# truongchauhien/CUDA.RadixSort

Measured on AMD Instinct MI355X. Metric: Mkeys/s sorting 2^30 uniform uint32; scatter-pass achieved HBM GB/s, higher is better.
Workload: dtype u32; 1 GPU; sort 1073741824 uint32 keys per GPU, k=8 (4 passes), uniform; keys_per_gpu=1073741824, k_bits=8, passes=4, dist=uniform, pairs=False, rank_algo=match, tile_keys=16384, tiles_per_chunk=256, num_chunks=256, parallelism=single GPU

## Files before the change

cuda.radixsort_amd/csrc/rsort_capi.cpp:

```cpp
#include <hip/hip_runtime.h>
#include <stdint.h>
#include <stdlib.h>
#include <string.h>

#include <math.h>

#include <algorithm>
#include <atomic>
#include <mutex>
#include <vector>

#include "rsort.h"
#include "rsort_internal.hpp"

using namespace rsort;

namespace {

constexpr int kVersion = 100;
std::atomic<int> g_rank_algo{RSORT_RANK_MATCH};
std::atomic<int> g_group_chunks{1};
std::atomic<int> g_table_fault{0};
std::atomic<int> g_rank_fault{0};
std::atomic<int> g_hybrid{RSORT_HYBRID_AUTO};
// ... 352 lines not shown
    a.kout = kout;
    a.vout = vout;
    a.table = table;
    a.n = (uint64_t)p.n;
    a.chunk_keys = (uint64_t)p.chunk_keys;
    a.num_chunks = (uint32_t)p.num_chunks;
    a.shift = (uint32_t)shift;
    a.local_only = local_only ? 1u : 0u;
    a.nsplit = (uint32_t)nsplit;
    for (int i = 0; i < nsplit; ++i) a.splitters[i] = split[i];
    const int rank = internal_rank((dmode == kDigitShift) ? g_rank_algo.load() : RSORT_RANK_MATCH);
    const int geom = geom_from_shape(p.threads, p.tile_keys, p.pairs);
    if (!scatter_available(p.k_bits, p.pairs, rank, dmode, geom)) return RSORT_ERR_ARG;
    const int aligned16 = line_capable(kout, vout, p.pairs, p.n);
    if ((bounds || next_table || raw_table) && !(rank == kRankAtomic && aligned16 && !local_only && dmode == kDigitShift))
        return RSORT_ERR_ARG;
    PhaseScope ps(dmode == kDigitSplit ? RSORT_PHASE_PARTITION : RSORT_PHASE_SCATTER, p.n, s, gate);
    return hip_status(launch_scatter(p.k_bits, p.pairs, rank, dmode, geom, local_only ? 0 : aligned16, a, s));
}

int check_plan(const rsort_plan *p) {
    if (!p) return RSORT_ERR_ARG;
    if (p->k_bits < kMinBits || p->k_bits > kMaxBits) return RSORT_ERR_BITS;
    if (p->n < 0 || p->n >= ((int64_t)1 << 32)) return RSORT_ERR_SIZE;
    if (geom_from_shape(p->threads, p->tile_keys, p->pairs) < 0) return RSORT_ERR_ARG;
    if (p->tiles_per_chunk <= 0 || p->num_chunks <= 0 ||
        p->num_chunks * p->tiles_per_chunk * p->tile_keys < p->n ||
        p->chunk_keys != p->tiles_per_chunk * p->tile_keys || p->bins != (1 << p->k_bits) ||
        p->table_entries != (int64_t)p->bins * p->num_chunks)
        return RSORT_ERR_ARG;
    return RSORT_OK;
}

constexpr int64_t kHybMinKeys = (int64_t)3 << 28;
constexpr int64_t kHybMaxKeys = (int64_t)kHybCapacity * kHybBuckets;
int64_t hyb_min_keys() {
    static const int64_t v = [] {
        const char *e = lab_env("RSORT_HYB_MIN_KEYS");
        const long long x = e ? atoll(e) : 0;
        return (x >= 1 && x < ((long long)1 << 32)) ? (int64_t)x : kHybMinKeys;
    }();
    return v;
}

constexpr int kHybGridMult = 4;

uint32_t gate_threshold(int64_t n) {
    const double m = (double)std::min<int64_t>(n, kHybSample) / (double)kHybGateGroups;
    const double lam = m * std::max(1.0 / (double)kHybBuckets, (double)kHybCapacity / (double)std::max<int64_t>(n, 1));
    double lp = -lam;
    for (uint32_t k = 0; k < 65535u; ++k) {
        if ((double)(k + 1) > lam) {
            const double tail = exp(lp) / (1.0 - lam / (double)(k + 1));
            if (tail * (double)kHybBuckets * (double)kHybGateGroups < 1e-9) return std::max(k, 2u);
        }
        lp += log(lam) - log((double)(k + 1));
    }
    return 65535u;
}

bool hybrid_eligible(const rsort_plan &p, bool joint, bool inplace, bool allow) {
    const int hm = g_hybrid.load();
    if (!allow || hm == RSORT_HYBRID_OFF || !joint || p.pairs || inplace || p.passes != 4) return false;
    if (hm == RSORT_HYBRID_FORCE) return true;
    return p.n >= hyb_min_keys() && p.n <= kHybMaxKeys;
}

int sort_planned(const rsort_plan &p, const uint32_t *kin, const uint32_t *vin, uint32_t *kout,
                 uint32_t *vout, void *ws, size_t wsb, hipStream_t s, bool allow_hybrid = true) {
    int st = check_plan(&p);
    if (st) return st;
    if (p.n == 0) return RSORT_OK;
    if (!kin || !kout || !ws || (p.pairs && (!vin || !vout))) return RSORT_ERR_ARG;
    if (!aligned4(kin) || !aligned4(kout) || (p.pairs && (!aligned4(vin) || !aligned4(vout))))
        return RSORT_ERR_ALIGN;
    if (wsb < p.workspace_bytes) return RSORT_ERR_WORKSPACE;
    const Carve c = carve(p, ws);
    const int P = p.passes;
// ... 32 lines not shown
        h.kin = kin;
        h.kout = kout;
        h.joint = c.joint;
        h.bounds = hb;
        h.gflags = c.bounds;
        h.done = c.done;
        h.n = (uint64_t)p.n;
        h.threshold = gate_threshold(p.n);
        h.force = force ? 1u : 0u;
        h.rank_fault = g_rank_fault.load() ? 1u : 0u;
        hyb_note_bucket();
        {
            PhaseScope ps(RSORT_PHASE_HISTOGRAM, std::min<int64_t>(p.n, kHybSample), s);
            if (hipMemsetAsync(c.joint, 0, (size_t)kJointBins * kJointBins * 4 + 16, s) != hipSuccess) return RSORT_ERR_HIP;
            if ((st = hip_status(launch_hyb_gate(h, s)))) return st;
        }
        if ((st = do_histogram_joint(p, kin, 24, c.table, c.joint, nullptr, s, false, nullptr, nullptr, nullptr, 16,
                                     g_try)))
            return st;
        {
            PhaseScope ps(RSORT_PHASE_HISTOGRAM, p.n, s);
            if ((st = hip_status(launch_hyb_bounds(h, s)))) return st;
        }
        if ((st = do_scan(p, c.table, c.bsums, s, nullptr, nullptr, nullptr, nullptr, g_run))) return st;
        if ((st = do_scatter(p, kin, nullptr, kout, nullptr, 24, c.table, 0, kDigitShift, nullptr, 0, s, nullptr,
                             nullptr, nullptr, nullptr, nullptr, 0, nullptr, c.done + kDoneErr, g_run)))
            return st;
        if ((st = do_scatter(p, kout, nullptr, c.tmp_k, nullptr, 16, c.joint, 0, kDigitShift, nullptr, 0, s, hb,
                             nullptr, nullptr, nullptr, nullptr, 0, nullptr, c.done + kDoneErr, g_run)))
            return st;
        {
            const int cus = std::max(1, device_cus());
            const int bpc = std::max(1, hyb_blocks_per_cu());
            const uint32_t grid = (uint32_t)std::min<int64_t>(kHybBuckets, (int64_t)cus * bpc * kHybGridMult);
            h.kin = c.tmp_k;
            PhaseScope ps(RSORT_PHASE_SCATTER, p.n, s, g_run);
            if ((st = hip_status(launch_hyb_bucket(h, grid, s)))) return st;
        }
    }
    for (int i = 0; i < P; ++i) {
        const int shift = i * p.k_bits;
        const bool to_out = ((P - 1 - i) % 2) == 0;
        uint32_t *dk = to_out ? kout : c.tmp_k;
        uint32_t *dv = to_out ? vout : c.tmp_v;
        const bool count_joint = joint && (i % 2 == 0) && i + 1 < P;
        const uint32_t *bounds = (joint && (i % 2 == 1)) ? c.bounds + (i / 2) * kBoundsWords : nullptr;
        uint32_t *tab = rawt ? rot[i % 3] : (nextc && (i % 2 == 1)) ? c.table2 : c.table;
        uint32_t *nxt = (nextc && i + 1 < P) ? (rawt ? rot[(i + 1) % 3] : (i % 2 == 1) ? c.table : c.table2) : nullptr;
        uint32_t *clr = (rawt && i + 2 < P) ? rot[(i + 2) % 3] : nullptr;
        const uint32_t *enable = (count_joint && i >= 2) ? c.bounds + (i / 2 - 1) * kBoundsWords : nullptr;
        if (count_joint) {
            if ((st = do_histogram_joint(p, sk, shift, c.table, c.joint, enable, s, i == 0 && !hyb, rows, rows_cnt,
                                         (i == 0 && !hyb) ? c.done : nullptr, 0, lsd)))
                return st;
        } else if (!(nextc && i > 0) &&
                   (st = do_histogram(p, sk, shift, tab, kDigitShift, nullptr, 0, s, bounds, c.joint, c.plan,
                                      c.pcounts, rawt ? nxt : nullptr, i == 0 ? c.done : nullptr,
                                      bounds ? rows : nullptr, lsd))) {
            return st;
        }
        if (!(nextc && i > 0) && !rawt &&
            (st = do_scan(p, tab, c.bsums, s, nxt, nextc ? c.done : nullptr, bounds ? &c : nullptr, bounds, lsd)))
            return st;
        if (count_joint && (st = do_joint_bounds(p, c.joint, enable, c.bounds + (i / 2) * kBoundsWords, c.plan,
                                                 c.pcounts, tab, rows_cnt, rows ? rows + kRowsWords : nullptr, s, lsd)))
            return st;
        const uint32_t *cl = (joint && i >= 1) ? c.bounds + ((i - 1) / 2) * kBoundsWords : nullptr;
// ... 405 lines not shown
    if (!d_keys_in || !d_keys_out || (plan->pairs && (!d_vals_in || !d_vals_out)))
        return RSORT_ERR_ARG;
    if (d_keys_in == d_keys_out) return RSORT_ERR_ARG;
    const uint32_t *table = nullptr;
    return do_scatter(*plan, d_keys_in, d_vals_in, d_keys_out, d_vals_out, shift, table, 1,
                      kDigitShift, nullptr, 0, (hipStream_t)stream);
}

int rsort_set_rank_algo(int algo) {
    if (algo != RSORT_RANK_MATCH && algo != RSORT_RANK_SPLIT && algo != RSORT_RANK_BALLOT) return RSORT_ERR_ARG;
    g_rank_algo.store(algo);
    return RSORT_OK;
}

int rsort_get_rank_algo(void) { return g_rank_algo.load(); }

int rsort_set_group_chunks(int enable) {
    g_group_chunks.store(enable ? 1 : 0);
    return RSORT_OK;
}

int rsort_get_group_chunks(void) { return g_group_chunks.load(); }

int rsort_set_hybrid(int mode) {
    if (mode != RSORT_HYBRID_AUTO && mode != RSORT_HYBRID_OFF && mode != RSORT_HYBRID_FORCE) return RSORT_ERR_ARG;
    g_hybrid.store(mode);
    return RSORT_OK;
}

int rsort_get_hybrid(void) { return g_hybrid.load(); }

int rsort_hybrid_capacity(void) { return (int)kHybCapacity; }

int rsort_hybrid_range(int64_t *min_keys, int64_t *max_keys) {
    if (!min_keys || !max_keys) return RSORT_ERR_ARG;
    *min_keys = hyb_min_keys();
    *max_keys = kHybMaxKeys;
    return RSORT_OK;
}

int rsort_hybrid_gate_threshold(int64_t n) {
    if (n <= 0 || n >= ((int64_t)1 << 32)) return -RSORT_ERR_SIZE;
    return (int)gate_threshold(n);
}

int rsort_hybrid_report(const rsort_plan *plan, const void *d_workspace, int *report, void *stream) {
    if (!plan || !report || !d_workspace) return RSORT_ERR_ARG;
    int st = check_plan(plan);
    if (st) return st;
    for (int i = 0; i < 4; ++i) report[i] = 0;
    if (plan->n == 0) return RSORT_OK;
    const Carve c = carve(*plan, const_cast<void *>(d_workspace));
    hipStream_t s = (hipStream_t)stream;
    uint32_t h[4] = {0, 0, 0, 0};
    if (hipMemcpyAsync(h, c.done + kHybMode, sizeof(h), hipMemcpyDeviceToHost, s) != hipSuccess) return RSORT_ERR_HIP;
    if (hipStreamSynchronize(s) != hipSuccess) return RSORT_ERR_HIP;
    report[0] = (int)h[kHybEligible - kHybMode];
    report[1] = (int)h[kHybGate - kHybMode];
    report[2] = (int)h[kHybMax - kHybMode];
    report[3] = h[0] == kHybRun ? 1 : 0;
    return RSORT_OK;
}

int rsort_group_flags(const rsort_plan *plan, const void *d_workspace, int *flags, void *stream) {
    if (!plan || !flags || !d_workspace) return RSORT_ERR_ARG;
    int st = check_plan(plan);
// ... 269 lines not shown
```

cuda.radixsort_amd/csrc/rsort_hooks.hpp:

```cpp
#pragma once
#include <hip/hip_runtime.h>
#include <stdint.h>

#ifdef RSORT_LAB_HOOKS
#include RSORT_LAB_HOOKS
#else
namespace rsort {
namespace hooks {
constexpr int kDeferKeysCl = 2;
constexpr int kDeferKeysPlain = 0;
constexpr int kDeferPairs = 4;
constexpr int kNextReplicas = 8;
constexpr int kLinesMinWavesSmall = 1;

typedef uint32_t u32x4h __attribute__((ext_vector_type(4)));
__device__ __forceinline__ void store_quad_nt(uint32_t *p, const u32x4h &v) {
    __builtin_nontemporal_store(v, reinterpret_cast<u32x4h *>(p));
}
__device__ __forceinline__ void store_quad(uint32_t *p, const u32x4h &v) { *reinterpret_cast<u32x4h *>(p) = v; }
__device__ __forceinline__ void store_word(uint32_t *p, uint32_t v) { *p = v; }
}
}
#define RS_WG_T0
#define RS_WG_T1
#define RS_WG_TH1
#define RS_STAMP_DECL
#define RS_STAMP(i)
#define RS_STAMP_FLUSH()
#endif
```

cuda.radixsort_amd/csrc/rsort_hybrid.hip:

```cpp
#include <hip/hip_runtime.h>
#include <stdint.h>

#include "rsort_device.hpp"
#include "rsort_hooks.hpp"
#include "rsort_internal.hpp"

namespace rsort {

namespace {

constexpr uint32_t kPadKey = 0xFFFFFFFFu;
typedef uint32_t u32x4 __attribute__((ext_vector_type(4)));

__global__ __launch_bounds__(1024) void rs_hyb_gate(HybArgs a) {
    constexpr uint32_t T = 1024;
    __shared__ uint32_t s_c[kHybBuckets / 2];
    const uint32_t t = threadIdx.x;
    const uint64_t m = a.n < (uint64_t)kHybSample ? a.n : (uint64_t)kHybSample;
    const uint64_t stride = m ? a.n / m : 1;
    const uint64_t i = (uint64_t)blockIdx.x * T + t;
    const uint32_t k = i < m ? __builtin_nontemporal_load(a.kin + i * stride) : 0u;
    for (uint32_t x = t; x < kHybBuckets / 2; x += T) s_c[x] = 0u;
    __syncthreads();
    if (i < m) {
        const uint32_t bk = k >> 16, sh = (bk & 1u) << 4;
        const uint32_t before = (atomicAdd(&s_c[bk >> 1], 1u << sh) >> sh) & 0xFFFFu;
        if (before + 1u >= a.threshold) a.joint[kHybGateFlag] = 1u;
    }
}

__global__ __launch_bounds__(1024) void rs_hyb_bounds(HybArgs a) {
    constexpr uint32_t R = kJointBins, Q = 1024 / R, EP = R / Q;
    __shared__ uint32_t s_part[Q][R];
    __shared__ uint32_t s_start[R];
    __shared__ uint32_t s_ws[1024 / kWave];
    __shared__ uint32_t s_max;
    const uint32_t t = threadIdx.x;
    const bool skew = a.joint[kHybGateFlag] != 0u;
    if (t == 0) {
        a.done[0] = 0u;
        a.done[kDoneErr] = 0u;
        a.done[kHybGate] = skew ? kGateSkewed : kGatePass;
        a.done[kHybEligible] = 1u;
    }
// ... 42 lines not shown
        }
        return;
    }
    if (t < R) {
        s_start[t] = start;
        a.bounds[1 + t] = start;
    }
    if (t == 0) {
        a.bounds[0] = kGroupsWhole;
        a.bounds[1 + R] = total;
    }
    __syncthreads();
    uint32_t run = s_start[g];
    for (uint32_t i = 0; i < q; ++i) run += s_part[i][g];
#pragma unroll 1
    for (uint32_t i0 = 0; i0 < EP; i0 += B) {
        uint32_t v[B];
#pragma unroll
        for (uint32_t i = 0; i < B; ++i) v[i] = col[(i0 + i) * R];
#pragma unroll
        for (uint32_t i = 0; i < B; ++i) {
            col[(i0 + i) * R] = run;
            run += v[i];
        }
    }
    if (t == 0) {
        a.done[kHybMode] = kHybRun;
        a.done[kHybMax] = big;
        a.gflags[0] = kGroupsWhole;
        a.gflags[kBoundsWords] = kGroupsFixed;
    }
}

template <int THREADS, int KPT>
__global__ __launch_bounds__(THREADS) void rs_bucket_sort16(HybArgs a) {
    constexpr int W = THREADS / kWave;
    constexpr uint32_t CAP = THREADS * KPT;
    static_assert(CAP == kHybCapacity && CAP % kWave == 0, "the capacity the exact count checks");
    __shared__ __attribute__((aligned(16))) uint32_t s_k[CAP + 4];
    __shared__ uint32_t s_cnt[W * 256];
    __shared__ uint32_t s_ws[W];
    if (a.done[kHybMode] != kHybRun) return;
    const uint32_t t = threadIdx.x, w = t / kWave, lane = lane_id();
    uint32_t *row = &s_cnt[w * 256];
    uint32_t order_bad = 0, size_bad = 0;
    auto bucket = [&](uint32_t b, uint32_t &s, uint32_t &n) {
        s = 0u;
        n = 0u;
        if (b >= kHybBuckets) return;
        s = a.joint[(b & 255u) * kJointBins + (b >> 8)];
        const uint32_t b1 = b + 1u;
        const uint32_t e = b1 < kHybBuckets ? a.joint[(b1 & 255u) * kJointBins + (b1 >> 8)] : (uint32_t)a.n;
        n = e - s;
        if (e < s || n > CAP || (uint64_t)e > a.n) {
            size_bad = 1u;
            n = 0u;
        }
    };
    auto span_of = [&](uint32_t n) { return ((((n + 63u) / 64u) + W - 1) / W) * 64u; };
    uint32_t key[KPT];
    auto load = [&](uint32_t s, uint32_t n) {
        const uint32_t span = span_of(n), i0 = w * span + lane;
#pragma unroll
        for (int j = 0; j < KPT; ++j) {
            const uint32_t i = i0 + j * kWave;
            const bool in = (uint32_t)(j * kWave) < span && i < n;
            key[j] = in ? __builtin_nontemporal_load(a.kin + s + i) : kPadKey;
        }
    };
    for (uint32_t b = blockIdx.x; b < kHybBuckets; b += gridDim.x) {
        uint32_t s, n;
        bucket(b, s, n);
        load(s, n);
        const uint32_t span = span_of(n), i0 = w * span + lane;
        const uint32_t ak = (uint32_t)(((uintptr_t)(a.kout + s) >> 2) & 3u);
        for (int pass = 0; pass < 2; ++pass) {
            const uint32_t sh = pass * 8;
            for (uint32_t i = lane; i < 256; i += kWave) row[i] = 0;
            uint32_t rk[KPT];
#pragma unroll
            for (int j = 0; j < KPT; ++j) {
                rk[j] = 0;
                if ((uint32_t)(j * kWave) < span && w * span + j * kWave < n) {
                    const uint32_t d = (key[j] >> sh) & 255u;
                    rk[j] = rank_add(row, d);
                    if (j == 0 && w * span + kWave <= n) order_bad |= rank_check<8>(d, rk[j], a.rank_fault);
                }
            }
            __syncthreads();
            uint32_t tot = 0;
            if (t < 256) {
#pragma unroll
                for (int x = 0; x < W; ++x) {
                    const uint32_t c = s_cnt[x * 256 + t];
                    s_cnt[x * 256 + t] = tot;
                    tot += c;
                }
            }
            uint32_t all;
            const uint32_t dbase = block_excl_scan<THREADS>(t < 256 ? tot : 0u, s_ws, all);
            if (t < 256) {
#pragma unroll
                for (int x = 0; x < W; ++x) s_cnt[x * 256 + t] += dbase;
            }
            __syncthreads();
#pragma unroll
            for (int j = 0; j < KPT; ++j) {
                if ((uint32_t)(j * kWave) < span && w * span + j * kWave < n) {
                    const uint32_t p = row[(key[j] >> sh) & 255u] + rk[j];
                    s_k[ak + p] = key[j];
                }
            }
            if (pass == 0) {
                __syncthreads();
#pragma unroll
                for (int j = 0; j < KPT; ++j) {
                    if ((uint32_t)(j * kWave) < span && w * span + j * kWave < n) key[j] = s_k[ak + i0 + j * kWave];
                }
            }
            __syncthreads();
        }
        {
            uint32_t *o = a.kout + s - ak;
            const uint32_t nq = (ak + n + 3u) / 4u;
            for (uint32_t q = t; q < nq; q += THREADS) {
                const u32x4 v = *reinterpret_cast<const u32x4 *>(&s_k[4 * q]);
                if (4 * q >= ak && 4 * q + 4 <= ak + n) {
                    hooks::store_quad_nt(o + 4 * q, v);
                } else {
#pragma unroll
                    for (uint32_t i = 0; i < 4; ++i)
                        if (4 * q + i >= ak && 4 * q + i < ak + n) hooks::store_word(o + 4 * q + i, v[i]);
                }
            }
        }
        __syncthreads();
    }
    if (a.done != nullptr && __ballot(size_bad != 0u) != 0ull && lane == 0) atomicOr(a.done + kDoneErr, kCheckTable);
    report_order(a.done + kDoneErr, order_bad);
}

const void *bucket_kernel() { return (const void *)rs_bucket_sort16<kHybThreads, kHybKpt>; }

}

hipError_t launch_hyb_gate(const HybArgs &a, hipStream_t s) {
    hipLaunchKernelGGL(rs_hyb_gate, dim3(kHybGateGroups), dim3(1024), 0, s, a);
    return hipGetLastError();
}

hipError_t launch_hyb_bounds(const HybArgs &a, hipStream_t s) {
    hipLaunchKernelGGL(rs_hyb_bounds, dim3(1), dim3(1024), 0, s, a);
    return hipGetLastError();
}

hipError_t launch_hyb_bucket(const HybArgs &a, uint32_t grid, hipStream_t s) {
    if (grid == 0) return hipErrorInvalidValue;
    const void *fn = bucket_kernel();
    HybArgs args = a;
    void *params[] = {&args};
    return hipLaunchKernel(fn, dim3(grid), dim3(kHybThreads), params, 0, s);
}

void hyb_note_bucket() {
    note_kernel_used(bucket_kernel(), "rs_bucket_sort16<1024, 18>");
}

int hyb_blocks_per_cu() {
    int nb = 0;
    if (hipOccupancyMaxActiveBlocksPerMultiprocessor(&nb, bucket_kernel(), kHybThreads, 0) != hipSuccess) return 0;
    return nb;
}

}
```

cuda.radixsort_amd/csrc/rsort_internal.hpp:

```cpp
#pragma once
#include <hip/hip_runtime.h>
#include <stdint.h>
#include <stdlib.h>

namespace rsort {

constexpr int kWave = 64;
constexpr int kHistThreads = 256;
constexpr int kMinBits = 1;
constexpr int kMaxBits = 13;
constexpr int kScanThreads = 256;
constexpr int kScanPerThread = 16;
constexpr int kScanSegment = kScanThreads * kScanPerThread;
constexpr int kMaxSplitters = 31;

enum DigitMode : int { kDigitShift = 0, kDigitSplit = 1 };

enum Geom : int { kGeomSmall = 0, kGeomLarge = 1, kGeomK4 = 2, kGeomLines = 3, kGeomLinesPairs = 4, kGeomXL = 5,
                  kGeomCount = 6 };
struct GeomShape {
    int threads;
    int kpt;
};
constexpr GeomShape kGeomShape[kGeomCount] = {{256, 16}, {512, 32}, {512, 16}, {1024, 16}, {1024, 8}, {128, 32}};
// ... 112 lines not shown
                               uint32_t snap, uint32_t weighted, hipStream_t s,
                               const uint32_t *ctab = nullptr, uint32_t *rows_cnt = nullptr,
                               const uint32_t *rowone = nullptr, const uint32_t *mode = nullptr,
                               uint32_t mode_want = 0);
hipError_t launch_scatter(int bits, int pairs, int rank_algo, int dmode, int geom, int aligned16,
                          const ScatterArgs &a, hipStream_t s);
bool scatter_available(int bits, int pairs, int rank_algo, int dmode, int geom);
hipError_t launch_scan(const ScanArgs &a, hipStream_t s);
hipError_t launch_gather_starts(const uint32_t *table, uint32_t num_chunks, uint32_t bins,
                                uint64_t n, uint32_t *starts, hipStream_t s);
hipError_t launch_diff_starts(const uint32_t *starts, uint32_t bins, uint32_t *hist,
                              hipStream_t s);
hipError_t launch_top_hist_sampled(const uint32_t *keys, uint64_t n, uint32_t top_bits, uint32_t stride,
                                   uint32_t *hist, hipStream_t s);
hipError_t launch_sample(const uint32_t *keys, uint64_t n, uint64_t stride, uint64_t count, uint64_t row_len,
                         uint32_t *out, hipStream_t s);
hipError_t launch_fingerprint(const uint32_t *keys, const uint32_t *vals, uint64_t n, unsigned long long *out,
                              hipStream_t s);
hipError_t launch_gen_uniform(uint32_t *out, uint64_t n, uint64_t seed, hipStream_t s);
hipError_t launch_gen_zipf(uint32_t *out, uint64_t n, uint64_t seed, const uint32_t *cdf,
                           uint64_t ranks, hipStream_t s);
hipError_t launch_gen_iota(uint32_t *out, uint64_t n, uint32_t base, hipStream_t s);
hipError_t launch_widen(const uint32_t *in, unsigned long long *out, uint32_t n, hipStream_t s);
int scatter_blocks_per_cu(int bits, int pairs, int rank_algo, int geom, int dmode = kDigitShift);
size_t scatter_kernels_used(char *buf, size_t len, int reset);
void note_kernel_used(const void *fn, const char *name);
void profile_pause(int delta);
constexpr uint32_t kDoneErr = 1;
constexpr uint32_t kCheckTable = 1u, kCheckRankOrder = 2u;

constexpr uint32_t kHybMode = 4, kHybGate = 5, kHybMax = 6, kHybEligible = 7;
constexpr uint32_t kHybLsd = 0, kHybRun = 2;
constexpr uint32_t kGateNone = 0, kGatePass = 1, kGateSkewed = 2;
constexpr int kHybThreads = 1024, kHybKpt = 18;
constexpr uint32_t kHybCapacity = kHybThreads * kHybKpt;
constexpr uint32_t kHybBuckets = kJointBins * kJointBins;
constexpr uint32_t kHybSample = 65536;
constexpr uint32_t kHybGateGroups = 64;
constexpr uint32_t kHybGateFlag = kJointBins * kJointBins + 1;
struct HybArgs {
    const uint32_t *kin;
    uint32_t *kout;
    uint32_t *joint;
    uint32_t *bounds;
    uint32_t *gflags;
    uint32_t *done;
    uint64_t n;
    uint32_t threshold;
    uint32_t force;
    uint32_t rank_fault;
};
hipError_t launch_hyb_gate(const HybArgs &a, hipStream_t s);
hipError_t launch_hyb_bounds(const HybArgs &a, hipStream_t s);
hipError_t launch_hyb_bucket(const HybArgs &a, uint32_t grid, hipStream_t s);
void hyb_note_bucket();
int hyb_blocks_per_cu();

constexpr int kSegWaveKpt = 4;
constexpr int kSegSmallThreads = 256, kSegSmallKpt = 4;
constexpr int kSegLdsThreads = 1024, kSegLdsKpt = 16;
constexpr int kSegWaveKeys = kWave * kSegWaveKpt;
constexpr int kSegSmallKeys = kSegSmallThreads * kSegSmallKpt;
constexpr int kSegLdsKeys = kSegLdsThreads * kSegLdsKpt;
enum SegKind : int { kSegWave = 0, kSegSmall = 1, kSegLds = 2, kSegTiles = 3, kSegRejected = 4, kSegKinds = 4 };
constexpr uint32_t kSegCheckWord = 8;
constexpr uint32_t kCheckOffsets = 4u;
struct SegClassifyArgs {
    const uint32_t *off;
    uint32_t *lists[kSegKinds];
    uint32_t *counters;
    uint64_t n;
    uint32_t num_segments;
};
struct SegSortArgs {
    const uint32_t *kin;
    const uint32_t *vin;
    uint32_t *kout;
    uint32_t *vout;
    uint32_t *ktmp;
    uint32_t *vtmp;
    const uint32_t *off;
    const uint32_t *list;
    const uint32_t *count;
    uint32_t *check;
    uint32_t rank_fault;
};
hipError_t launch_seg_classify(const SegClassifyArgs &a, hipStream_t s);
hipError_t launch_seg_sort(int kind, int pairs, int rank_algo, const SegSortArgs &a, uint32_t grid, hipStream_t s);
int seg_blocks_per_cu(int kind, int pairs, int rank_algo);
// ... 9 lines not shown
```

cuda.radixsort_amd/radixsort.py:

```python
from __future__ import annotations

import ctypes
import enum
import os
import time
from contextlib import contextmanager
from pathlib import Path

import numpy as np

try:
    import torch
except Exception:
    torch = None

PKG = Path(__file__).resolve().parent
LIB_PATH = PKG / "librsort.so"

RSORT_OK = 0
STATUS_NAMES = {0: "RSORT_OK", 1: "RSORT_ERR_ARG", 2: "RSORT_ERR_BITS", 3: "RSORT_ERR_SIZE",
                4: "RSORT_ERR_ALIGN", 5: "RSORT_ERR_ALLOC", 6: "RSORT_ERR_HIP",
                7: "RSORT_ERR_WORKSPACE", 8: "RSORT_ERR_NODEV", 9: "RSORT_ERR_CAPACITY",
                10: "RSORT_ERR_COMM", 11: "RSORT_ERR_CHECK"}
RANK_MATCH, RANK_SPLIT, RANK_BALLOT = 0, 1, 2
# ... 89 lines not shown

class MultiStats(ctypes.Structure):
    _fields_ = [("world", ctypes.c_int32), ("rank", ctypes.c_int32), ("halves", ctypes.c_int32),
                ("direct", ctypes.c_int32), ("rounds", ctypes.c_int64), ("bytes_per_key", ctypes.c_int64),
                ("send_keys", ctypes.c_int64 * MAX_RANKS), ("recv_keys", ctypes.c_int64 * MAX_RANKS),
                ("n_in", ctypes.c_int64), ("n_out", ctypes.c_int64),
                ("ms_plan", ctypes.c_double), ("ms_partition", ctypes.c_double), ("ms_exchange", ctypes.c_double),
                ("ms_local_sort", ctypes.c_double), ("ms_total", ctypes.c_double)]

    def as_dict(self):
        w = self.world
        d = {f: getattr(self, f) for f, _ in self._fields_ if f not in ("send_keys", "recv_keys")}
        d["send_keys"] = [int(self.send_keys[i]) for i in range(w)]
        d["recv_keys"] = [int(self.recv_keys[i]) for i in range(w)]
        return d


_u32p, _vp, _i64, _int, _sz = (ctypes.POINTER(ctypes.c_uint32), ctypes.c_void_p, ctypes.c_int64,
                               ctypes.c_int, ctypes.c_size_t)
_i = _int
_PP = ctypes.POINTER(Plan)
SIGNATURES = {
    "rsort_status_string": ([_int], ctypes.c_char_p),
    "rsort_version": ([], _int),
    "rsort_plan_make": ([_i64, _int, _int, _i64, _PP], _int),
    "rsort_workspace_size": ([_i64, _int, _int], _sz),
    "rsort_u32_device": ([_vp, _vp, _i64, _int, _vp, _sz, _vp], _int),
    "rsort_u32_pairs_device": ([_vp, _vp, _vp, _vp, _i64, _int, _vp, _sz, _vp], _int),
    "rsort_sort_planned": ([_PP, _vp, _vp, _vp, _vp, _vp, _sz, _vp], _int),
    "rsort_sort_planned_ex": ([_PP, _vp, _vp, _vp, _vp, _vp, _sz, _vp, _int], _int),
    "rsort_set_hybrid": ([_int], _int),
    "rsort_get_hybrid": ([], _int),
    "rsort_hybrid_capacity": ([], _int),
    "rsort_hybrid_range": ([ctypes.POINTER(_i64), ctypes.POINTER(_i64)], _int),
    "rsort_hybrid_gate_threshold": ([_i64], _int),
    "rsort_hybrid_report": ([ctypes.c_void_p, ctypes.c_void_p, ctypes.c_void_p, ctypes.c_void_p], _int),
    "rsort_u32": ([_vp, _vp, _i64, _int], _int),
    "rsort_u32_ex": ([_vp, _vp, _i64, _int, _int, ctypes.POINTER(PhaseTimes)], _int),
    "rsort_u32_pairs": ([_vp, _vp, _vp, _vp, _i64, _int], _int),
    "rsort_pass_histogram": ([_PP, _vp, _int, _vp, _vp], _int),
    "rsort_pass_scan": ([_PP, _vp, _vp, _vp], _int),
    "rsort_pass_scatter": ([_PP, _vp, _vp, _vp, _vp, _int, _vp, _vp], _int),
    "rsort_pass_local_sort": ([_PP, _vp, _vp, _vp, _vp, _int, _vp], _int),
    "rsort_set_rank_algo": ([_int], _int),
    "rsort_get_rank_algo": ([], _int),
    "rsort_set_group_chunks": ([_int], _int),
    "rsort_get_group_chunks": ([], _int),
    "rsort_group_flags": ([ctypes.c_void_p, ctypes.c_void_p, ctypes.c_void_p, ctypes.c_void_p], _int),
    "rsort_lane_order_probe": ([], _int),
    "rsort_plan_check": ([ctypes.c_void_p, ctypes.c_void_p, ctypes.c_void_p, ctypes.c_void_p], _int),
    "rsort_cut_plan_stats": ([ctypes.c_void_p, ctypes.c_void_p, ctypes.c_void_p, ctypes.c_void_p], _int),
    "rsort_plan_features": ([_PP], _int),
    "rsort_inject_table_fault": ([_int], _int),
    "rsort_inject_rank_fault": ([_int], _int),
    "rsort_scatter_kernels_used": ([ctypes.c_char_p, _sz, _int], _sz),
    "rsort_profile_begin": ([], _int),
    "rsort_profile_end": ([ctypes.POINTER(PhaseTimes)], _int),
    "rsort_partition_workspace_size": ([_i64, _int, _int], _sz),
    "rsort_partition_device": ([_vp, _vp, _vp, _vp, _i64, _u32p, _int, _vp, _vp, _sz, _vp], _int),
    "rsort_partition_check": ([_i64, _int, _int, _vp, ctypes.c_void_p, _vp], _int),
    "rsort_top_histogram": ([_vp, _i64, _int, _vp, _vp, _sz, _vp], _int),
    "rsort_top_histogram_sampled": ([_vp, _i64, _int, _int, _vp, _vp], _int),
    "rsort_multi_workspace_size": ([_i64, _i64, _int, _int, _int], _sz),
    "rsort_u32_multi": ([_vp, _vp, _i64, _vp, _vp, _i64, ctypes.POINTER(_i64), ctypes.POINTER(_i64), _int, _vp,
                         _vp, _sz, _vp], _int),
    "rsort_multi_sample_plan": ([_i, ctypes.POINTER(_i64), _i64, ctypes.POINTER(SamplePlan)], _int),
# ... 176 lines not shown
        _check(_lib().rsort_sort_planned_ex(ctypes.byref(p), _ptr(keys_in), _ptr(vals_in), _ptr(keys_out),
                                            _ptr(vals_out), _ptr(ws), ws.numel(), _stream(stream), SORT_NO_HYBRID),
               "rsort_sort_planned_ex")
    return keys_out


SORT_NO_HYBRID = 1
HYBRID_AUTO, HYBRID_OFF, HYBRID_FORCE = 0, 1, 2
GATE_NONE, GATE_PASS, GATE_SKEWED = 0, 1, 2


def set_hybrid(mode: int):
    _check(_lib().rsort_set_hybrid(int(mode)), "rsort_set_hybrid")


def get_hybrid() -> int:
    return int(_lib().rsort_get_hybrid())


@contextmanager
def hybrid(mode: int):
    old = get_hybrid()
    set_hybrid(mode)
    try:
        yield
    finally:
        set_hybrid(old)


def hybrid_capacity() -> int:
    return int(_lib().rsort_hybrid_capacity())


def hybrid_range() -> tuple[int, int]:
    lo, hi = _i64(), _i64()
    _check(_lib().rsort_hybrid_range(ctypes.byref(lo), ctypes.byref(hi)), "rsort_hybrid_range")
    return int(lo.value), int(hi.value)


def hybrid_gate_threshold(n: int) -> int:
    t = int(_lib().rsort_hybrid_gate_threshold(int(n)))
    if t < 0:
        raise RSortError(-t, "rsort_hybrid_gate_threshold")
    return t


def hybrid_report(p: Plan, ws, stream=None) -> dict:
    r = (ctypes.c_int * 4)()
    _check(_lib().rsort_hybrid_report(ctypes.byref(p), _ptr(ws), r, _stream(stream)), "rsort_hybrid_report")
    return {"eligible": bool(r[0]), "gate": int(r[1]), "max_bucket": int(r[2]), "hybrid": bool(r[3])}


def group_flags(p: Plan, ws, stream=None) -> list[int]:
    flags = (ctypes.c_int * 2)()
    _check(_lib().rsort_group_flags(ctypes.byref(p), _ptr(ws), flags, _stream(stream)), "rsort_group_flags")
    return [int(flags[0]), int(flags[1])]


def cut_plan_stats(p: Plan, ws, stream=None) -> list[dict]:
    st = (ctypes.c_int * 8)()
    _check(_lib().rsort_cut_plan_stats(ctypes.byref(p), _ptr(ws), st, _stream(stream)), "rsort_cut_plan_stats")
    keys = ("key_ranges", "row_tasks", "direct_adds", "negative_ranges")
    return [{k: int(st[4 * i + j]) for j, k in enumerate(keys)} for i in range(2)]


FEAT_GROUPS, FEAT_NEXT_DIGIT, FEAT_RAW_TABLES, FEAT_TAIL_SCAN = 1, 2, 4, 8
# ... 515 lines not shown
```

dev/lab_hooks.hpp:

```cpp
#pragma once
#include <hip/hip_runtime.h>
#include <stdint.h>

#ifndef RSORT_DEFER_KEYS_CL
#define RSORT_DEFER_KEYS_CL 2
#endif
#ifndef RSORT_DEFER_KEYS_PLAIN
#define RSORT_DEFER_KEYS_PLAIN 0
#endif
#ifndef RSORT_DEFER_PAIRS
#define RSORT_DEFER_PAIRS 4
#endif
#ifndef RSORT_NXR
#define RSORT_NXR 8
#endif
#ifndef RSORT_LINES_MINW_SMALL
#define RSORT_LINES_MINW_SMALL 1
#endif

namespace rsort {
namespace hooks {
constexpr int kDeferKeysCl = RSORT_DEFER_KEYS_CL;
constexpr int kDeferKeysPlain = RSORT_DEFER_KEYS_PLAIN;
constexpr int kDeferPairs = RSORT_DEFER_PAIRS;
// ... 44 lines not shown
#define RS_WG_T1 RS_WG_TREC(g_wg_times, (a.shift / BITS) & 7u, 2048u, cbeg, cend)
#define RS_WG_TH1 RS_WG_TREC(g_wg_htimes, (a.shift / 8u) & 3u, 256u, beg, end)
extern "C" __attribute__((visibility("default"), used)) int rsort_lab_wg_times(unsigned long long *host) {
    return hipMemcpyFromSymbol(host, HIP_SYMBOL(rsort::g_wg_times), sizeof(rsort::g_wg_times)) == hipSuccess &&
                   hipMemcpyFromSymbol(host + 8 * 2048 * 4, HIP_SYMBOL(rsort::g_wg_htimes), sizeof(rsort::g_wg_htimes)) ==
                       hipSuccess
               ? 0
               : 6;
}
#else
#define RS_WG_T0
#define RS_WG_T1
#define RS_WG_TH1
#endif

#ifdef RSORT_STAMPS
#define RS_STAMP_DECL unsigned long long st_acc_[8] = {0, 0, 0, 0, 0, 0, 0, 0}, st_prev_ = __builtin_amdgcn_s_memtime();
#define RS_STAMP(i)                                                   \
    do {                                                              \
        const unsigned long long now_ = __builtin_amdgcn_s_memtime(); \
        st_acc_[i] += now_ - st_prev_;                                \
        st_prev_ = now_;                                              \
    } while (0)
#define RS_STAMP_FLUSH()                                                                   \
    do {                                                                                   \
        if (threadIdx.x == 0 && a.stamps)                                                  \
            for (int i_ = 0; i_ < 8; ++i_) a.stamps[blockIdx.x * 8 + i_] = st_acc_[i_];    \
    } while (0)
#else
#define RS_STAMP_DECL
#define RS_STAMP(i)
#define RS_STAMP_FLUSH()
#endif
```

include/rsort.h:

```cpp
#ifndef RSORT_H_
#define RSORT_H_

#include <stddef.h>
#include <stdint.h>

#ifdef __cplusplus
extern "C" {
#endif

#if defined(_WIN32)
#define RSORT_API
#else
#define RSORT_API __attribute__((visibility("default")))
#endif

typedef enum rsort_status {
    RSORT_OK = 0,
    RSORT_ERR_ARG = 1,
    RSORT_ERR_BITS = 2,
    RSORT_ERR_SIZE = 3,
    RSORT_ERR_ALIGN = 4,
    RSORT_ERR_ALLOC = 5,
    RSORT_ERR_HIP = 6,
    RSORT_ERR_WORKSPACE = 7,
// ... 74 lines not shown
RSORT_API int    rsort_u32_segmented_device(const uint32_t *d_keys_in, const uint32_t *d_vals_in,
                                            uint32_t *d_keys_out, uint32_t *d_vals_out, int64_t n,
                                            const uint32_t *d_offsets, int64_t num_segments,
                                            void *d_workspace, size_t workspace_bytes, void *stream);
#define RSORT_CHECK_OFFSETS 4
RSORT_API int    rsort_segmented_check(int64_t n, int64_t num_segments, int pairs, const void *d_workspace,
                                       int *flags, int64_t *class_counts, void *stream);
RSORT_API int    rsort_u32_segmented(const uint32_t *keys_in, const uint32_t *vals_in, uint32_t *keys_out,
                                     uint32_t *vals_out, int64_t n, const uint32_t *offsets,
                                     int64_t num_segments);

RSORT_API int rsort_pass_histogram(const rsort_plan *plan, const uint32_t *d_keys, int shift,
                                   uint32_t *d_table, void *stream);
RSORT_API int rsort_pass_scan(const rsort_plan *plan, uint32_t *d_table, uint32_t *d_block_sums,
                              void *stream);
RSORT_API int rsort_pass_scatter(const rsort_plan *plan, const uint32_t *d_keys_in,
                                 const uint32_t *d_vals_in, uint32_t *d_keys_out,
                                 uint32_t *d_vals_out, int shift, const uint32_t *d_table,
                                 void *stream);
RSORT_API int rsort_pass_local_sort(const rsort_plan *plan, const uint32_t *d_keys_in,
                                    const uint32_t *d_vals_in, uint32_t *d_keys_out,
                                    uint32_t *d_vals_out, int shift, void *stream);

RSORT_API int rsort_set_rank_algo(int algo);
RSORT_API int rsort_get_rank_algo(void);
RSORT_API int rsort_set_group_chunks(int enable);
RSORT_API int rsort_get_group_chunks(void);
#define RSORT_HYBRID_AUTO 0
#define RSORT_HYBRID_OFF 1
#define RSORT_HYBRID_FORCE 2
RSORT_API int rsort_set_hybrid(int mode);
RSORT_API int rsort_get_hybrid(void);
RSORT_API int rsort_hybrid_capacity(void);
RSORT_API int rsort_hybrid_range(int64_t *min_keys, int64_t *max_keys);
RSORT_API int rsort_hybrid_gate_threshold(int64_t n);
#define RSORT_GATE_NONE 0
#define RSORT_GATE_PASS 1
#define RSORT_GATE_SKEWED 2
RSORT_API int rsort_hybrid_report(const rsort_plan *plan, const void *d_workspace, int *report, void *stream);
RSORT_API int rsort_group_flags(const rsort_plan *plan, const void *d_workspace, int *flags,
                                void *stream);
RSORT_API int rsort_cut_plan_stats(const rsort_plan *plan, const void *d_workspace, int *stats, void *stream);
#define RSORT_CHECK_TABLE 1
#define RSORT_CHECK_RANK_ORDER 2
RSORT_API int rsort_plan_check(const rsort_plan *plan, const void *d_workspace, int *flags, void *stream);
#define RSORT_FEAT_GROUPS 1
#define RSORT_FEAT_NEXT_DIGIT 2
#define RSORT_FEAT_RAW_TABLES 4
#define RSORT_FEAT_TAIL_SCAN 8
RSORT_API int rsort_plan_features(const rsort_plan *plan);
RSORT_API int rsort_inject_table_fault(int enable);
RSORT_API int rsort_inject_rank_fault(int enable);
RSORT_API size_t rsort_scatter_kernels_used(char *buf, size_t len, int reset);
RSORT_API int rsort_lane_order_probe(void);
RSORT_API int rsort_profile_begin(void);
RSORT_API int rsort_profile_end(rsort_phase_times *out);

RSORT_API size_t rsort_partition_workspace_size(int64_t n, int num_buckets, int pairs);
RSORT_API int rsort_partition_device(const uint32_t *d_keys_in, const uint32_t *d_vals_in,
                                     uint32_t *d_keys_out, uint32_t *d_vals_out, int64_t n,
                                     const uint32_t *splitters, int num_buckets,
                                     uint32_t *d_bucket_starts, void *d_workspace,
                                     size_t workspace_bytes, void *stream);
RSORT_API int rsort_partition_check(int64_t n, int num_buckets, int pairs, const void *d_workspace, int *flags,
                                    void *stream);
RSORT_API int rsort_top_histogram(const uint32_t *d_keys, int64_t n, int top_bits,
// ... 130 lines not shown
```

Measured before the change: 142,000 Mkeys/s.

## Pack hybrid bucket-sort keys into 16-bit LDS tiles and raise occupancy

The hybrid bucket-sort kernel now keeps only the low 16 bits of each key in registers and LDS, packing two keys per register, and rebuilds the high bits from the bucket index when storing. The key tile in LDS is halved, the launch bounds request two resident blocks per CU, the block scan becomes a wave scan over 256 digit columns, and uniform scalar slot counts replace per-key bounds checks. The grid multiplier doubles to 8 and is overridable by an environment variable, and the minimum size for the hybrid path drops. It adds a check that every loaded key matches its bucket's high bits, plus stamp hooks and a kernel-info API for profiling.

Result: faster. 170,700 Mkeys/s (median of 6 runs) (+20.2%).

```diff
diff --git a/cuda.radixsort_amd/csrc/rsort_capi.cpp b/cuda.radixsort_amd/csrc/rsort_capi.cpp
--- a/cuda.radixsort_amd/csrc/rsort_capi.cpp
+++ b/cuda.radixsort_amd/csrc/rsort_capi.cpp
@@ -408,7 +408,7 @@
     return RSORT_OK;
 }
 
-constexpr int64_t kHybMinKeys = (int64_t)3 << 28;
+constexpr int64_t kHybMinKeys = (int64_t)1 << 28;
 constexpr int64_t kHybMaxKeys = (int64_t)kHybCapacity * kHybBuckets;
 int64_t hyb_min_keys() {
     static const int64_t v = [] {
@@ -419,7 +419,15 @@
     return v;
 }
 
-constexpr int kHybGridMult = 4;
+constexpr int kHybGridMult = 8;
+int hyb_grid_mult() {
+    static const int v = [] {
+        const char *e = lab_env("RSORT_HYB_GRID_MULT");
+        const int x = e ? atoi(e) : 0;
+        return (x >= 1 && x <= 256) ? x : kHybGridMult;
+    }();
+    return v;
+}
 
 uint32_t gate_threshold(int64_t n) {
     const double m = (double)std::min<int64_t>(n, kHybSample) / (double)kHybGateGroups;
@@ -518,7 +526,7 @@
         {
             const int cus = std::max(1, device_cus());
             const int bpc = std::max(1, hyb_blocks_per_cu());
-            const uint32_t grid = (uint32_t)std::min<int64_t>(kHybBuckets, (int64_t)cus * bpc * kHybGridMult);
+            const uint32_t grid = (uint32_t)std::min<int64_t>(kHybBuckets, (int64_t)cus * bpc * hyb_grid_mult());
             h.kin = c.tmp_k;
             PhaseScope ps(RSORT_PHASE_SCATTER, p.n, s, g_run);
             if ((st = hip_status(launch_hyb_bucket(h, grid, s)))) return st;
@@ -990,6 +998,11 @@
 
 int rsort_hybrid_capacity(void) { return (int)kHybCapacity; }
 
+int rsort_hybrid_kernel_info(int *info) {
+    if (!info) return RSORT_ERR_ARG;
+    return hyb_kernel_info(info) == hipSuccess ? RSORT_OK : RSORT_ERR_HIP;
+}
+
 int rsort_hybrid_range(int64_t *min_keys, int64_t *max_keys) {
     if (!min_keys || !max_keys) return RSORT_ERR_ARG;
     *min_keys = hyb_min_keys();
diff --git a/cuda.radixsort_amd/csrc/rsort_hooks.hpp b/cuda.radixsort_amd/csrc/rsort_hooks.hpp
--- a/cuda.radixsort_amd/csrc/rsort_hooks.hpp
+++ b/cuda.radixsort_amd/csrc/rsort_hooks.hpp
@@ -27,4 +27,9 @@
 #define RS_STAMP_DECL
 #define RS_STAMP(i)
 #define RS_STAMP_FLUSH()
+#define RS_HYB_STAMP_DECL
+#define RS_HYB_STAMP(i)
+#define RS_HYB_STAMP_LOADED(i)
+#define RS_HYB_STAMP_BUCKET()
+#define RS_HYB_STAMP_FLUSH()
 #endif
diff --git a/cuda.radixsort_amd/csrc/rsort_hybrid.hip b/cuda.radixsort_amd/csrc/rsort_hybrid.hip
--- a/cuda.radixsort_amd/csrc/rsort_hybrid.hip
+++ b/cuda.radixsort_amd/csrc/rsort_hybrid.hip
@@ -1,5 +1,6 @@
 #include <hip/hip_runtime.h>
 #include <stdint.h>
+#include <stdio.h>
 
 #include "rsort_device.hpp"
 #include "rsort_hooks.hpp"
@@ -9,7 +10,6 @@
 
 namespace {
 
-constexpr uint32_t kPadKey = 0xFFFFFFFFu;
 typedef uint32_t u32x4 __attribute__((ext_vector_type(4)));
 
 __global__ __launch_bounds__(1024) void rs_hyb_gate(HybArgs a) {
@@ -118,99 +118,147 @@
     }
 }
 
+__device__ __forceinline__ uint32_t fresh_scalar(uint32_t x) {
+    x = __builtin_amdgcn_readfirstlane(x);
+    asm volatile("" : "+s"(x));
+    return x;
+}
+__device__ __forceinline__ uint32_t fresh_vector(uint32_t x) {
+    asm volatile("" : "+v"(x));
+    return x;
+}
+
 template <int THREADS, int KPT>
-__global__ __launch_bounds__(THREADS) void rs_bucket_sort16(HybArgs a) {
-    constexpr int W = THREADS / kWave;
+__global__ __launch_bounds__(THREADS, kHybResident *THREADS / 256) void rs_bucket_sort16(HybArgs a) {
+    constexpr int W = THREADS / kWave, KP = KPT / 2, SW = 256 / kWave;
     constexpr uint32_t CAP = THREADS * KPT;
     static_assert(CAP == kHybCapacity && CAP % kWave == 0, "the capacity the exact count checks");
-    __shared__ __attribute__((aligned(16))) uint32_t s_k[CAP + 4];
+    static_assert(KPT % 2 == 0 && KPT * kWave <= 65536 && CAP <= 65536, "ranks and positions in 16 bits");
+    static_assert(THREADS >= 256, "one thread per digit in the column prefix");
+    __shared__ __attribute__((aligned(16))) uint16_t s_k[CAP + 8];
     __shared__ uint32_t s_cnt[W * 256];
-    __shared__ uint32_t s_ws[W];
+    __shared__ uint32_t s_ws[SW];
     if (a.done[kHybMode] != kHybRun) return;
-    const uint32_t t = threadIdx.x, w = t / kWave, lane = lane_id();
+    RS_HYB_STAMP_DECL
+    const uint32_t t = threadIdx.x, lane = lane_id();
+    const uint32_t w = __builtin_amdgcn_readfirstlane(t / kWave);
     uint32_t *row = &s_cnt[w * 256];
-    uint32_t order_bad = 0, size_bad = 0;
-    auto bucket = [&](uint32_t b, uint32_t &s, uint32_t &n) {
-        s = 0u;
-        n = 0u;
-        if (b >= kHybBuckets) return;
-        s = a.joint[(b & 255u) * kJointBins + (b >> 8)];
+    uint32_t order_bad = 0, table_bad = 0;
+    for (uint32_t b = blockIdx.x; b < kHybBuckets; b += gridDim.x) {
+        const uint32_t s = a.joint[(b & 255u) * kJointBins + (b >> 8)];
         const uint32_t b1 = b + 1u;
         const uint32_t e = b1 < kHybBuckets ? a.joint[(b1 & 255u) * kJointBins + (b1 >> 8)] : (uint32_t)a.n;
-        n = e - s;
+        uint32_t n = e - s;
         if (e < s || n > CAP || (uint64_t)e > a.n) {
-            size_bad = 1u;
+            table_bad = 1u;
             n = 0u;
         }
-    };
-    auto span_of = [&](uint32_t n) { return ((((n + 63u) / 64u) + W - 1) / W) * 64u; };
-    uint32_t key[KPT];
-    auto load = [&](uint32_t s, uint32_t n) {
-        const uint32_t span = span_of(n), i0 = w * span + lane;
-#pragma unroll
-        for (int j = 0; j < KPT; ++j) {
-            const uint32_t i = i0 + j * kWave;
-            const bool in = (uint32_t)(j * kWave) < span && i < n;
-            key[j] = in ? __builtin_nontemporal_load(a.kin + s + i) : kPadKey;
-        }
-    };
-    for (uint32_t b = blockIdx.x; b < kHybBuckets; b += gridDim.x) {
-        uint32_t s, n;
-        bucket(b, s, n);
-        load(s, n);
-        const uint32_t span = span_of(n), i0 = w * span + lane;
+        const uint32_t span = ((((n + 63u) / 64u) + W - 1) / W) * 64u, base = w * span;
+        const uint32_t slots0 = base < n ? (min(span, n - base) + 63u) / 64u : 0u;
+        const bool full0 = base + kWave <= n;
+        const uint32_t hi = b << 16;
+        uint32_t key[KP];
+        {
+            const uint32_t left = base < n ? n - base : 0u;
+            const uint32_t *in = a.kin + s + base;
+            const uint32_t slots = fresh_scalar(slots0), ll = fresh_vector(lane);
+            uint32_t diff = 0;
+#pragma unroll
+            for (int i = 0; i < KP; ++i) {
+                uint32_t k[2] = {hi | 0xFFFFu, hi | 0xFFFFu};
+#pragma unroll
+                for (int h = 0; h < 2; ++h) {
+                    const uint32_t j = 2 * i + h, x = j * kWave + ll;
+                    if (j < slots) {
+                        const uint32_t v = __builtin_nontemporal_load(in + min(x, left - 1u));
+                        k[h] = x < left ? v : k[h];
+                    }
+                    diff |= k[h] ^ hi;
+                }
+                key[i] = (k[0] & 0xFFFFu) | (k[1] << 16);
+            }
+            table_bad |= diff >> 16;
+            asm volatile("" : "+v"(table_bad));
+        }
+        RS_HYB_STAMP_LOADED(0);
         const uint32_t ak = (uint32_t)(((uintptr_t)(a.kout + s) >> 2) & 3u);
+        uint16_t *tile = s_k + ak;
+#pragma unroll 1
         for (int pass = 0; pass < 2; ++pass) {
             const uint32_t sh = pass * 8;
             for (uint32_t i = lane; i < 256; i += kWave) row[i] = 0;
-            uint32_t rk[KPT];
-#pragma unroll
-            for (int j = 0; j < KPT; ++j) {
-                rk[j] = 0;
-                if ((uint32_t)(j * kWave) < span && w * span + j * kWave < n) {
-                    const uint32_t d = (key[j] >> sh) & 255u;
-                    rk[j] = rank_add(row, d);
-                    if (j == 0 && w * span + kWave <= n) order_bad |= rank_check<8>(d, rk[j], a.rank_fault);
+            uint32_t rk[KP];
+            uint32_t slots = fresh_scalar(slots0);
+#pragma unroll
+            for (int i = 0; i < KP; ++i) {
+                rk[i] = 0;
+#pragma unroll
+                for (int h = 0; h < 2; ++h) {
+                    const uint32_t j = 2 * i + h;
+                    if (j < slots) {
+                        const uint32_t d = (key[i] >> (16 * h + sh)) & 255u;
+                        uint32_t r = rank_add(row, d);
+                        if (j == 0 && full0) order_bad |= rank_check<8>(d, r, a.rank_fault);
+                        rk[i] |= r << (16 * h);
+                    }
                 }
             }
             __syncthreads();
-            uint32_t tot = 0;
+            uint32_t c[W], tot = 0;
             if (t < 256) {
 #pragma unroll
                 for (int x = 0; x < W; ++x) {
-                    const uint32_t c = s_cnt[x * 256 + t];
+                    c[x] = s_cnt[x * 256 + t];
+                    tot += c[x];
+                }
+                const uint32_t inc = wave_incl_scan(tot);
+                if (lane == kWave - 1) s_ws[w] = inc;
+                tot = inc - tot;
+            }
+            __syncthreads();
+            if (t < 256) {
+#pragma unroll
+                for (int x = 0; x < SW; ++x) tot += (uint32_t)x < w ? s_ws[x] : 0u;
+#pragma unroll
+                for (int x = 0; x < W; ++x) {
                     s_cnt[x * 256 + t] = tot;
-                    tot += c;
-                }
-            }
-            uint32_t all;
-            const uint32_t dbase = block_excl_scan<THREADS>(t < 256 ? tot : 0u, s_ws, all);
-            if (t < 256) {
-#pragma unroll
-                for (int x = 0; x < W; ++x) s_cnt[x * 256 + t] += dbase;
+                    tot += c[x];
+                }
             }
             __syncthreads();
-#pragma unroll
-            for (int j = 0; j < KPT; ++j) {
-                if ((uint32_t)(j * kWave) < span && w * span + j * kWave < n) {
-                    const uint32_t p = row[(key[j] >> sh) & 255u] + rk[j];
-                    s_k[ak + p] = key[j];
-                }
-            }
+            slots = fresh_scalar(slots0);
+#pragma unroll
+            for (int i = 0; i < KP; ++i) {
+#pragma unroll
+                for (int h = 0; h < 2; ++h) {
+                    const uint32_t j = 2 * i + h;
+                    if (j < slots) {
+                        const uint32_t kh = key[i] >> (16 * h);
+                        const uint32_t p = row[(kh >> sh) & 255u] + ((rk[i] >> (16 * h)) & 0xFFFFu);
+                        tile[p] = (uint16_t)kh;
+                    }
+                }
+            }
+            __syncthreads();
             if (pass == 0) {
-                __syncthreads();
-#pragma unroll
-                for (int j = 0; j < KPT; ++j) {
-                    if ((uint32_t)(j * kWave) < span && w * span + j * kWave < n) key[j] = s_k[ak + i0 + j * kWave];
-                }
-            }
-            __syncthreads();
+                const uint16_t *mine = tile + base + lane;
+                slots = fresh_scalar(slots0);
+#pragma unroll
+                for (int i = 0; i < KP; ++i) {
+                    uint32_t lo = 0xFFFFu, up = 0xFFFFu;
+                    if ((uint32_t)(2 * i) < slots) lo = mine[(2 * i) * kWave];
+                    if ((uint32_t)(2 * i + 1) < slots) up = mine[(2 * i + 1) * kWave];
+                    key[i] = lo | (up << 16);
+                }
+            }
+            RS_HYB_STAMP(1 + pass);
         }
         {
             uint32_t *o = a.kout + s - ak;
             const uint32_t nq = (ak + n + 3u) / 4u;
-            for (uint32_t q = t; q < nq; q += THREADS) {
-                const u32x4 v = *reinterpret_cast<const u32x4 *>(&s_k[4 * q]);
+            for (uint32_t q = fresh_vector(t); q < nq; q += THREADS) {
+                const uint2 h2 = *reinterpret_cast<const uint2 *>(&s_k[4 * q]);
+                const u32x4 v = {hi | (h2.x & 0xFFFFu), hi | (h2.x >> 16), hi | (h2.y & 0xFFFFu), hi | (h2.y >> 16)};
                 if (4 * q >= ak && 4 * q + 4 <= ak + n) {
                     hooks::store_quad_nt(o + 4 * q, v);
                 } else {
@@ -220,9 +268,11 @@
                 }
             }
         }
-        __syncthreads();
-    }
-    if (a.done != nullptr && __ballot(size_bad != 0u) != 0ull && lane == 0) atomicOr(a.done + kDoneErr, kCheckTable);
+        RS_HYB_STAMP(3);
+        RS_HYB_STAMP_BUCKET();
+    }
+    RS_HYB_STAMP_FLUSH();
+    if (a.done != nullptr && __ballot(table_bad != 0u) != 0ull && lane == 0) atomicOr(a.done + kDoneErr, kCheckTable);
     report_order(a.done + kDoneErr, order_bad);
 }
 
@@ -249,7 +299,9 @@
 }
 
 void hyb_note_bucket() {
-    note_kernel_used(bucket_kernel(), "rs_bucket_sort16<1024, 18>");
+    char name[48];
+    snprintf(name, sizeof(name), "rs_bucket_sort16<%d, %d>", kHybThreads, kHybKpt);
+    note_kernel_used(bucket_kernel(), name);
 }
 
 int hyb_blocks_per_cu() {
@@ -258,4 +310,15 @@
     return nb;
 }
 
-}
+hipError_t hyb_kernel_info(int info[4]) {
+    hipFuncAttributes fa{};
+    const hipError_t e = hipFuncGetAttributes(&fa, bucket_kernel());
+    if (e != hipSuccess) return e;
+    info[0] = kHybThreads;
+    info[1] = (int)fa.sharedSizeBytes;
+    info[2] = (int)fa.localSizeBytes;
+    info[3] = hyb_blocks_per_cu();
+    return hipSuccess;
+}
+
+}
diff --git a/cuda.radixsort_amd/csrc/rsort_internal.hpp b/cuda.radixsort_amd/csrc/rsort_internal.hpp
--- a/cuda.radixsort_amd/csrc/rsort_internal.hpp
+++ b/cuda.radixsort_amd/csrc/rsort_internal.hpp
@@ -168,7 +168,7 @@
 constexpr uint32_t kHybMode = 4, kHybGate = 5, kHybMax = 6, kHybEligible = 7;
 constexpr uint32_t kHybLsd = 0, kHybRun = 2;
 constexpr uint32_t kGateNone = 0, kGatePass = 1, kGateSkewed = 2;
-constexpr int kHybThreads = 1024, kHybKpt = 18;
+constexpr int kHybThreads = 1024, kHybKpt = 18, kHybResident = 2;
 constexpr uint32_t kHybCapacity = kHybThreads * kHybKpt;
 constexpr uint32_t kHybBuckets = kJointBins * kJointBins;
 constexpr uint32_t kHybSample = 65536;
@@ -191,6 +191,7 @@
 hipError_t launch_hyb_bucket(const HybArgs &a, uint32_t grid, hipStream_t s);
 void hyb_note_bucket();
 int hyb_blocks_per_cu();
+hipError_t hyb_kernel_info(int info[4]);
 
 constexpr int kSegWaveKpt = 4;
 constexpr int kSegSmallThreads = 256, kSegSmallKpt = 4;
diff --git a/cuda.radixsort_amd/radixsort.py b/cuda.radixsort_amd/radixsort.py
--- a/cuda.radixsort_amd/radixsort.py
+++ b/cuda.radixsort_amd/radixsort.py
@@ -145,6 +145,7 @@
     "rsort_set_hybrid": ([_int], _int),
     "rsort_get_hybrid": ([], _int),
     "rsort_hybrid_capacity": ([], _int),
+    "rsort_hybrid_kernel_info": ([ctypes.POINTER(_int)], _int),
     "rsort_hybrid_range": ([ctypes.POINTER(_i64), ctypes.POINTER(_i64)], _int),
     "rsort_hybrid_gate_threshold": ([_i64], _int),
     "rsort_hybrid_report": ([ctypes.c_void_p, ctypes.c_void_p, ctypes.c_void_p, ctypes.c_void_p], _int),
@@ -387,6 +388,12 @@
     return int(_lib().rsort_hybrid_capacity())
 
 
+def hybrid_kernel_info() -> dict:
+    v = (_int * 4)()
+    _check(_lib().rsort_hybrid_kernel_info(v), "rsort_hybrid_kernel_info")
+    return {"threads": int(v[0]), "lds_bytes": int(v[1]), "scratch_bytes": int(v[2]), "resident_per_cu": int(v[3])}
+
+
 def hybrid_range() -> tuple[int, int]:
     lo, hi = _i64(), _i64()
     _check(_lib().rsort_hybrid_range(ctypes.byref(lo), ctypes.byref(hi)), "rsort_hybrid_range")
diff --git a/dev/hyb_stamps.py b/dev/hyb_stamps.py
--- /dev/null
+++ b/dev/hyb_stamps.py
@@ -0,0 +1,50 @@
+import argparse
+import ctypes
+import json
+import sys
+from pathlib import Path
+
+sys.path.insert(0, str(Path(__file__).resolve().parent.parent / "cuda.radixsort_amd"))
+import radixsort as rs
+import torch
+
+PHASES = ["load_issue_and_wait", "pass0", "pass1", "store_issue"]
+
+
+def main():
+    ap = argparse.ArgumentParser()
+    ap.add_argument("--log2n", type=int, default=30)
+    ap.add_argument("--reps", type=int, default=5)
+    a = ap.parse_args()
+    n = 1 << a.log2n
+    lib = rs._lib()
+    read = lib.rsort_lab_hyb_stamps
+    read.argtypes = [ctypes.POINTER(ctypes.c_uint64)]
+    read.restype = ctypes.c_int
+    buf = (ctypes.c_uint64 * 8)()
+    p = rs.plan(n, 8)
+    keys, out = rs.empty_u32(n), rs.empty_u32(n)
+    ws = rs.workspace(p.workspace_bytes)
+    rs.gen_uniform(keys, 0x5EED)
+    with rs.hybrid(rs.HYBRID_FORCE):
+        rs.sort_device(keys, out, 8, ws=ws, plan_=p)
+        assert rs.hybrid_report(p, ws)["hybrid"] and rs.plan_check(p, ws) == 0
+        assert read(buf) == 0
+        e0, e1 = torch.cuda.Event(enable_timing=True), torch.cuda.Event(enable_timing=True)
+        e0.record()
+        for _ in range(a.reps):
+            rs.sort_device(keys, out, 8, ws=ws, plan_=p)
+        e1.record()
+        torch.cuda.synchronize()
+        assert read(buf) == 0
+    v = [int(x) for x in buf]
+    buckets = v[7]
+    res = {"log2n": a.log2n, "reps": a.reps, "buckets_stamped": buckets, "ms_per_sort_stamped_build": e0.elapsed_time(e1) / a.reps,
+           "cycles_per_bucket": {PHASES[i]: round(v[i] / buckets, 1) for i in range(4)},
+           "cycles_per_bucket_total": round(sum(v[:4]) / buckets, 1),
+           "kernels_used": rs.scatter_kernels_used()}
+    print(json.dumps(res))
+
+
+if __name__ == "__main__":
+    main()
diff --git a/dev/lab_hooks.hpp b/dev/lab_hooks.hpp
--- a/dev/lab_hooks.hpp
+++ b/dev/lab_hooks.hpp
@@ -100,3 +100,39 @@
 #define RS_STAMP(i)
 #define RS_STAMP_FLUSH()
 #endif
+
+#ifdef RSORT_HYB_STAMPS
+namespace rsort {
+__device__ unsigned long long g_hyb_stamps[8];
+}
+extern "C" __attribute__((visibility("default"), used)) int rsort_lab_hyb_stamps(unsigned long long *host) {
+    const unsigned long long zero[8] = {0, 0, 0, 0, 0, 0, 0, 0};
+    if (hipDeviceSynchronize() != hipSuccess) return 6;
+    if (hipMemcpyFromSymbol(host, HIP_SYMBOL(rsort::g_hyb_stamps), sizeof(zero)) != hipSuccess) return 6;
+    return hipMemcpyToSymbol(HIP_SYMBOL(rsort::g_hyb_stamps), zero, sizeof(zero)) == hipSuccess ? 0 : 6;
+}
+#define RS_HYB_STAMP_DECL unsigned long long hs_acc_[8] = {0, 0, 0, 0, 0, 0, 0, 0}, hs_prev_ = __builtin_amdgcn_s_memtime();
+#define RS_HYB_STAMP(i)                                               \
+    do {                                                              \
+        const unsigned long long now_ = __builtin_amdgcn_s_memtime(); \
+        hs_acc_[i] += now_ - hs_prev_;                                \
+        hs_prev_ = now_;                                              \
+    } while (0)
+#define RS_HYB_STAMP_LOADED(i)                                \
+    do {                                                      \
+        asm volatile("s_waitcnt vmcnt(0)" ::: "memory");      \
+        RS_HYB_STAMP(i);                                      \
+    } while (0)
+#define RS_HYB_STAMP_BUCKET() hs_acc_[7] += 1
+#define RS_HYB_STAMP_FLUSH()                                                                    \
+    do {                                                                                        \
+        if (threadIdx.x == 0)                                                                   \
+            for (int i_ = 0; i_ < 8; ++i_) atomicAdd(&rsort::g_hyb_stamps[i_], hs_acc_[i_]);    \
+    } while (0)
+#else
+#define RS_HYB_STAMP_DECL
+#define RS_HYB_STAMP(i)
+#define RS_HYB_STAMP_LOADED(i)
+#define RS_HYB_STAMP_BUCKET()
+#define RS_HYB_STAMP_FLUSH()
+#endif
diff --git a/include/rsort.h b/include/rsort.h
--- a/include/rsort.h
+++ b/include/rsort.h
@@ -130,6 +130,7 @@
 RSORT_API int rsort_set_hybrid(int mode);
 RSORT_API int rsort_get_hybrid(void);
 RSORT_API int rsort_hybrid_capacity(void);
+RSORT_API int rsort_hybrid_kernel_info(int *info);
 RSORT_API int rsort_hybrid_range(int64_t *min_keys, int64_t *max_keys);
 RSORT_API int rsort_hybrid_gate_threshold(int64_t n);
 #define RSORT_GATE_NONE 0
```
